# JeremyCCHsu/vae-npvc

Measured on AMD Instinct MI355X. Metric: SP frames/sec (train step: fwd+bwd+Adam), higher is better.
Workload: dtype f32 tensors and accumulation / bf16x2 operands (16 mantissa bits) on the matrix cores

## Files before the change

### include/vaenpvc.h

```cpp
#ifndef VAENPVC_H_
#define VAENPVC_H_

#include <stddef.h>
#include <stdint.h>

#ifdef __cplusplus
extern "C" {
#endif

#define VAENPVC_MAX_LAYERS 8

#define VAENPVC_OK 0
#define VAENPVC_E_ARG (-1)
#define VAENPVC_E_WORKSPACE (-2)
#define VAENPVC_E_HIP (-3)
#define VAENPVC_E_UNSUPPORTED (-4)
#define VAENPVC_E_STATE (-5)

#define VAENPVC_IMPL_AUTO 0
#define VAENPVC_IMPL_GENERIC 1

#define VAENPVC_MODE_INFER 0
#define VAENPVC_MODE_TRAIN 1

// ... 8 lines not shown
  int32_t y_dim;
  int32_t n_enc;
  int32_t enc_kernel[VAENPVC_MAX_LAYERS];
  int32_t enc_stride[VAENPVC_MAX_LAYERS];
  int32_t enc_output[VAENPVC_MAX_LAYERS];
  int32_t gen_h;
  int32_t gen_c;
  int32_t n_dec;
  int32_t dec_kernel[VAENPVC_MAX_LAYERS];
  int32_t dec_stride[VAENPVC_MAX_LAYERS];
  int32_t dec_output[VAENPVC_MAX_LAYERS];
} vaenpvc_arch;

typedef struct vaenpvc_ctx vaenpvc_ctx;

int vaenpvc_abi_version(void);
const char* vaenpvc_last_error(void);

int vaenpvc_ctx_create(const vaenpvc_arch* arch, vaenpvc_ctx** out);
void vaenpvc_ctx_destroy(vaenpvc_ctx* ctx);
int vaenpvc_set_impl(vaenpvc_ctx* ctx, int impl);
int vaenpvc_set_precision(vaenpvc_ctx* ctx, int planes);
int vaenpvc_get_precision(const vaenpvc_ctx* ctx);

int vaenpvc_param_count(const vaenpvc_ctx* ctx);
int64_t vaenpvc_param_floats(const vaenpvc_ctx* ctx);
int vaenpvc_param_info(const vaenpvc_ctx* ctx, int index, char* name, int name_cap,
                       int64_t* offset_floats, int32_t* ndim, int64_t* shape);

int64_t vaenpvc_workspace_bytes(const vaenpvc_ctx* ctx, int64_t F, int mode);
int vaenpvc_ws_find(const vaenpvc_ctx* ctx, int64_t F, int mode, const char* name,
                    int64_t* offset_floats, int64_t* count_floats);

int vaenpvc_encode_fwd(vaenpvc_ctx* ctx, const float* d_params, const float* d_x, int64_t F,
                       float* d_z_mu, float* d_z_lv, void* d_ws, size_t ws_bytes, void* stream);

int vaenpvc_decode_fwd(vaenpvc_ctx* ctx, const float* d_params, const float* d_z,
                       const int64_t* d_y, int64_t F, float* d_xh, void* d_ws, size_t ws_bytes,
                       void* stream);

int vaenpvc_train_fwd_bwd(vaenpvc_ctx* ctx, const float* d_params, const float* d_x,
                          const int64_t* d_y, const float* d_eps, int64_t F, float* d_grads,
                          float* d_loss3, void* d_ws, size_t ws_bytes, void* stream);

int vaenpvc_train_fwd_bwd_seeded(vaenpvc_ctx* ctx, const float* d_params, const float* d_x,
                                 const int64_t* d_y, uint64_t seed, uint64_t offset,
// ... 126 lines not shown
```

### vae-npvc_amd/csrc/abi.hip

```cpp
#include <climits>
#include <cmath>
#include <cstdarg>
#include <cstdio>
#include <cstring>
#include <map>
#include <memory>
#include <mutex>

#include "../../include/vaenpvc_debug.h"
#include "kernels.h"

using namespace vaenpvc;

typedef std::pair<std::vector<Region>, int64_t> Layout;
struct vaenpvc_ctx {
  Model m;
  int impl = VAENPVC_IMPL_AUTO;
  Runtime rt;
  std::recursive_mutex mu;
  std::map<std::pair<int64_t, int>, std::shared_ptr<const Layout>> ws_cache;
};
struct Call {
  std::lock_guard<std::recursive_mutex> lk;
  RtScope sc;
// ... 90 lines not shown

static bool use_tuned(const vaenpvc_ctx* c) {
  return c->impl == VAENPVC_IMPL_AUTO && c->m.is_vcc2016 && tuned::available();
}

extern "C" {

int vaenpvc_set_tuned_masks(vaenpvc_ctx* ctx, uint32_t fwd_mask, uint32_t bwd_mask) {
  if (!ctx) return fail(VAENPVC_E_ARG, "null context");
  Call call(ctx, false);
  ctx->rt.fwd_mask = fwd_mask;
  ctx->rt.bwd_mask = bwd_mask;
  return 0;
}

int vaenpvc_set_precision(vaenpvc_ctx* ctx, int planes) {
  if (!ctx || planes < 1 || planes > 3) return fail(VAENPVC_E_ARG, "precision must be 1, 2 or 3 bf16 terms");
  Call call(ctx, false);
  ctx->rt.planes = planes;
  return 0;
}
int vaenpvc_get_precision(const vaenpvc_ctx* ctx) { return ctx ? ctx->rt.planes : VAENPVC_E_ARG; }

int vaenpvc_set_bucket_callback(vaenpvc_ctx* ctx, vaenpvc_bucket_cb cb, void* user) {
  if (!ctx) return fail(VAENPVC_E_ARG, "null context");
  Call call(ctx, false);
  ctx->rt.bucket_cb = cb;
  ctx->rt.bucket_user = user;
  return 0;
}

int vaenpvc_timer_select(vaenpvc_ctx* ctx, const char* tag) {
  if (!ctx) return fail(VAENPVC_E_ARG, "null context");
  Call call(ctx, false);
  ctx->rt.tag = tag ? tag : "";
  ctx->rt.used = 0;
  return 0;
}

int vaenpvc_timer_read(vaenpvc_ctx* ctx, double* total_ms, int64_t* launches) {
  if (!ctx) return fail(VAENPVC_E_ARG, "null context");
  Call call(ctx, false);
  Runtime& r = ctx->rt;
  double tot = 0.0;
  for (size_t i = 0; i < r.used; ++i) {
    float ms = 0.f;
// ... 617 lines not shown
```

### vae-npvc_amd/csrc/gfx950_elem.h

```cpp
#pragma once
#include "gfx950_common.h"

namespace vaenpvc {
namespace tuned {

template <int N>
__global__ void __launch_bounds__(256) k_ln_stats_fast(const float* __restrict__ a, float* __restrict__ st, int F) {
  static_assert(N % 4 == 0, "frame size must be a multiple of 4 floats");
  constexpr int NV = N / 4, PER = cdiv(NV, 64);
  const int lane = threadIdx.x & 63;
  const int f = blockIdx.x * 4 + (threadIdx.x >> 6);
  if (f >= F) return;
  const float4* p = reinterpret_cast<const float4*>(a + (int64_t)f * N);
  float4 v[PER];
  float s = 0.f;
#pragma unroll
  for (int i = 0; i < PER; ++i) {
    int idx = lane + 64 * i;
    v[i] = idx < NV ? p[idx] : make_float4(0.f, 0.f, 0.f, 0.f);
    s += (v[i].x + v[i].y) + (v[i].z + v[i].w);
  }
  const float mean = wave_sum(s) / N;
  float q = 0.f;
#pragma unroll
// ... 729 lines not shown
    int yk[8];
#pragma unroll
    for (int u = 0; u < 8; ++u) {
      const int f = f0 + u < fe ? f0 + u : fe - 1;
      v[u] = f0 + u < fe ? d[(int64_t)f * N + nn] : 0.f;
      int64_t yy = y[f];
      yk[u] = (int)(yy < 0 ? 0 : (yy >= NY ? NY - 1 : yy));
    }
#pragma unroll
    for (int u = 0; u < 8; ++u) {
      const int ku = __builtin_amdgcn_readfirstlane(yk[u]);
#pragma unroll
      for (int k = 0; k < NY; ++k)
        if (ku == k) acc[k] += v[u];
    }
  }
  if (n < N) {
#pragma unroll
    for (int k = 0; k < NY; ++k)
      if (acc[k] != 0.f) atomicAdd(S + (int64_t)k * N + n, acc[k]);
  }
}

template <int NY>
__global__ void __launch_bounds__(256) k_merge_small(const float* __restrict__ S, const float* __restrict__ E,
                                                     const float* __restrict__ Wy, int zd, int M, float* __restrict__ dWy,
                                                     float* __restrict__ dE, float* __restrict__ db1, float* __restrict__ db2,
                                                     float* __restrict__ db3, int nb_w, int nb_e) {
  const int b = blockIdx.x, tid = threadIdx.x;
  if (b < nb_w) {
    const int i = b * 256 + tid;
    if (i >= zd * M) return;
    const int m = i / M, n = i - m * M;
    float acc = 0.f;
#pragma unroll
    for (int k = 0; k < NY; ++k) acc += E[k * zd + m] * S[(int64_t)k * M + n];
    dWy[i] = acc;
  } else if (b < nb_w + nb_e) {
    const int o = (b - nb_w) * 4 + (tid >> 6), lane = tid & 63;
    if (o >= NY * zd) return;
    const int k = o / zd, m = o - k * zd;
    float acc = 0.f;
    for (int n = lane; n < M; n += 64) acc += S[(int64_t)k * M + n] * Wy[(int64_t)m * M + n];
    acc = wave_sum(acc);
    if (lane == 0) dE[o] = acc;
  } else {
// ... 105 lines not shown
```

### vae-npvc_amd/csrc/gfx950_layers.hip

```cpp
#include <cstdlib>
#include <cstring>
#include <type_traits>

#include "gfx950_convgemm.h"
#include "gfx950_convwgrad.h"
#include "gfx950_dense.h"
#include "gfx950_elem.h"
#include "gfx950_tngemm.h"
#include "gfx950_toeplitz.h"
#include "gfx950_toep_bf16.h"
#include "gfx950_planegemm.h"
#include "gfx950_ntring.h"
#include "gfx950_viewconv.h"
#include "gfx950_fconv.h"
#include "gfx950_fwgrad.h"
#include "gfx950_fconv_r.h"
#include "gfx950_fbwd.h"
#include "gfx950_lnb_planes.h"
#include "kernels.h"

namespace vaenpvc {
namespace tuned {

#ifndef E1F_T
// ... 120 lines not shown
  static constexpr int gd2 = d2f + D2F::BTOTAL;
  static constexpr int gd0 = gd2 + GD2::BTOTAL;
  static constexpr int ge4 = gd0 + GD0::BTOTAL;
  static constexpr int ge3 = ge4 + GE4::BTOTAL;
  static constexpr int ge2 = ge3 + GE3::BTOTAL;
  static constexpr int ge1 = ge2 + GE2::BTOTAL;
  static constexpr int wc = ge1 + GE1::BTOTAL;
  static constexpr int lnpart = wc + TOEP_C * WROW;
  static constexpr int wdg = lnpart + 2048 * 3 * 256;
  static constexpr int wfw = wdg + TB_WFLOATS;
  static constexpr int heads_bias = wfw + TB_WFLOATS;
  static constexpr int pg_headsf = heads_bias + 256;
  static constexpr int pg_headsb = pg_headsf + 3 * 256 * 768 / 2;
  static constexpr int pg_mergef = pg_headsb + 3 * 768 * 256 / 2;
  static constexpr int pg_mergeb = pg_mergef + 3 * 1664 * 128 / 2;
  static constexpr int pg_enc4f = pg_mergeb + 3 * 128 * 1600 / 2;
  static constexpr int pg_enc4b = pg_enc4f + 3 * 768 * 896 / 2;
  static constexpr int pg_bias4 = pg_enc4b + 3 * 896 * 768 / 2;
  static constexpr int cvw = pg_bias4 + 768;
  static constexpr int cvwr_d0f = cvw + CV_WTOTAL;
  static constexpr int cvwr_e2g = cvwr_d0f + fcr_wfloats(CV_D0F);
  static constexpr int enc0part_ = cvwr_e2g + fcr_wfloats(CV_E2G);
  static constexpr int enc0part = enc0part_;
  static constexpr int total = enc0part + 512 * 7 * 16;
};
static_assert(Pk::total <= 8 * 939162 + 65536, "packed weights must fit the scratch region");
static inline bool sel(unsigned mask, int bit) { return (mask >> bit) & 1u; }
static inline bool fwd_on(int bit) { return sel(rt().fwd_mask, bit); }
static inline bool bwd_on(int bit) { return sel(rt().bwd_mask, bit); }
constexpr unsigned SEL_STEPS = (2u << VAENPVC_SEL_DEC3) - 1;
constexpr int64_t PLANEGEMM_MIN_FRAMES = 1024;
static inline bool pg_on(unsigned mask, int64_t F) {
  return sel(mask, VAENPVC_SEL_PLANE_GEMM) && (F >= PLANEGEMM_MIN_FRAMES || !sel(mask, VAENPVC_SEL_PLANE_GEMM_MIN_FRAMES));
}
static inline bool pg_fwd(int64_t F) { return pg_on(rt().fwd_mask, F); }
static inline bool cg_fwd(int64_t F) { return fwd_on(VAENPVC_SEL_VIEW_GEMM) && pg_on(rt().fwd_mask | (1u << VAENPVC_SEL_PLANE_GEMM), F); }
static inline bool cg_bwd(int64_t F) { return bwd_on(VAENPVC_SEL_VIEW_GEMM) && pg_on(rt().bwd_mask | (1u << VAENPVC_SEL_PLANE_GEMM), F); }
static inline bool pg_bwd(int64_t F) { return pg_on(rt().bwd_mask, F); }
static inline bool pg_step(int bit, int64_t F) { return bwd_on(bit) && pg_bwd(F) && pg_fwd(F) && fwd_on(bit); }
static inline bool cv_sel(unsigned mask, int site) { return !sel(mask, VAENPVC_SEL_CV_SITE_SET) || ((rt().cv_sites() >> site) & 1u); }
static inline bool cv_fwd(int site, int64_t F) { return cg_fwd(F) && cv_sel(rt().fwd_mask, site); }
static inline bool cv_bwd(int site, int64_t F) { return cg_bwd(F) && cv_sel(rt().bwd_mask, site); }
constexpr int64_t FCONV_MIN_FRAMES = 1024;
constexpr int64_t ENC0_WAVE_MIN_FRAMES = 1024;
static inline bool enc0_wave(unsigned mask, int64_t F) { return F >= ENC0_WAVE_MIN_FRAMES || !sel(mask, VAENPVC_SEL_ENC0_WAVE_MIN_FRAMES); }
static inline bool fc_on(unsigned mask, int site, int64_t F) {
  if (!fconv_serves(site, rt().planes)) return false;
// ... 18 lines not shown
  if (rt().planes > VAENPVC_FB_MAXPL || !bwd_on(VAENPVC_SEL_FBWD)) return false;
  if (!((rt().fb_layers() >> layer) & 1u)) return false;
  return F >= FCONV_MIN_FRAMES || !bwd_on(VAENPVC_SEL_FBWD_MIN_FRAMES);
}
static bool toep_bf16_for(int64_t F);
static inline bool act_bf16(int64_t F) {
  Runtime& r = rt();
  if (!r.act_bf16 || r.planes != 1 || F < FCONV_MIN_FRAMES) return false;
  const unsigned need = (1u << VAENPVC_SEL_DEC1) | (1u << VAENPVC_SEL_DEC2) | (1u << VAENPVC_SEL_DEC3);
  if ((r.fwd_mask & need) != need || (r.bwd_mask & need) != need) return false;
  return fc_fwd(CV_D1F, F) && fc_fwd(CV_D2F, F) && toep_bf16_for(F) && fb_bwd(FB_D2, F) && fb_bwd(FB_D1, F);
}
static inline bool fc_any(int64_t F) {
  for (int i = 0; i < CV_COUNT; ++i)
    if (fc_fwd(i, F) || fc_bwd(i, F) || fcr_fwd(i, F) || fcr_bwd(i, F)) return true;
  return false;
}
static inline bool fwd_planes(int bit, int site, int64_t F) {
  return fwd_on(bit) && cv_fwd(site, F) && !fc_fwd(site, F) && !fcr_fwd(site, F);
}
static inline bool cw_bwd(int site, int64_t F) { return cg_bwd(F) && cv_sel(rt().bwd_mask, CV_COUNT + site); }
static inline bool d0f_leaves_planes(int64_t F) {
  return F >= 1024 && fwd_on(VAENPVC_SEL_DEC0) && fcr_fwd(CV_D0F, F) && bwd_on(VAENPVC_SEL_DEC0) && cw_bwd(CW_D0, F);
}
static inline unsigned short* us(float* p) { return reinterpret_cast<unsigned short*>(p); }
static NtArgs nt_args(const float* Ap, int M, int Kp, const float* Bp, int Np, int N, float* C, int ldc) {
  NtArgs a;
  memset(&a, 0, sizeof a);
  a.A = reinterpret_cast<const unsigned short*>(Ap);
  a.B = reinterpret_cast<const unsigned short*>(Bp);
  a.a_plane = (int64_t)M * Kp;
  a.b_plane = (int64_t)Np * Kp;
  a.M = M;
  a.N = N;
  a.Kp = Kp;
  a.C = C;
  a.ldc = ldc;
  return a;
}
#ifndef TN_WGS_DENSE
#define TN_WGS_DENSE 384
#endif
static TnpArgs tnp_args(const float* Ap, int lda, const float* Bp, int ldb, int M, int N, int F, float* C, int ldc) {
  TnpArgs a;
  memset(&a, 0, sizeof a);
  a.A = reinterpret_cast<const unsigned short*>(Ap);
// ... 305 lines not shown
    a.beta = P + m.enc[4].beta_off;
    a.out2 = w.z_lv;
    a.split = 128;
    a.bias = w.scratch + Pk::heads_bias;
    if (F < SMALL_BATCH_FRAMES) {
      if (w.z_lv == w.z_mu + (size_t)F * 128) {
        (void)hipMemsetAsync(w.z_mu, 0, (size_t)F * 256 * 4, s);
      } else {
        (void)hipMemsetAsync(w.z_mu, 0, (size_t)F * 128 * 4, s);
        (void)hipMemsetAsync(w.z_lv, 0, (size_t)F * 128 * 4, s);
      }
      VAENPVC_TIMED("heads_fwd", s, launch_densegemm<HeadsFs>(a, s, 6));
    } else
    VAENPVC_TIMED("heads_fwd", s, launch_densegemm<HeadsF>(a, s));
  } else generic::heads_fwd(m, P, F, w, s);
}

void decoder_fwd(const Model& m, const float* P, const float* z, const int64_t* y, int64_t F64, const Ws& w,
                 float* xh_out, hipStream_t s, bool weights_packed) {
  const int F = (int)F64;
  if (!weights_packed) prep(m, P, w, F, s);
  const bool z_planes_done = rt().plz_F == F && z == w.z;
  rt().plz_F = -1;
  if (fwd_on(VAENPVC_SEL_MERGE) && pg_fwd(F)) {
    for_planes([&](auto npl) {
      constexpr int NPL = decltype(npl)::value;
      if (!z_planes_done) VAENPVC_TIMED("merge_split", s, launch_split<NPL>(split_args(z, 128, 128, F, us(w.pl_z)), s));
      NtArgs a = nt_args(w.pl_z, F, 128, w.scratch + Pk::pg_mergef, 1664, 1539, w.h, 1539);
      a.rowbias = w.scratch + Pk::merge_tb;
      a.idx = y;
      a.nrb = MERGE_NY;
      a.ldrb = 1539;
      VAENPVC_TIMED("merge_fwd", s, launch_gemm_nt<NPL>(a, s));
    });
  } else if (fwd_on(VAENPVC_SEL_MERGE)) {
    DenseArgs a = dense_args(z, w.scratch + Pk::merge_f, w.h, m.merge, F);
    a.idx = y;
    a.rowbias = w.scratch + Pk::merge_tb;
    a.nrb = MERGE_NY;
    VAENPVC_TIMED("merge_fwd", s, (F < SMALL_BATCH_FRAMES ? launch_densegemm<MergeFs>(a, s) : launch_densegemm<MergeF>(a, s)));
  } else generic::merge_fwd(m, P, z, y, F, w, s);
  const bool abf = act_bf16(F);
  auto fused = [&](int site, const float* src, const float* st, float* st_out, const ConvL* ln, const float* bias, float* out, const char* tag,
                   bool bf_in = false, bool bf_out = false) {
    for_planes([&](auto npl) {
      FcArgs fa{src, st, st_out, ln ? P + ln->gamma_off : nullptr, ln ? P + ln->beta_off : nullptr,
// ... 7 lines not shown
    for_planes([&](auto npl) {
      constexpr int NPL = decltype(npl)::value;
      if (have) {}
      else if (i == 0) VAENPVC_TIMED(tsplit, s, cv_split<NPL>(cl, src, nullptr, nullptr, nullptr, w.cl[cl], F, s));
      else VAENPVC_TIMED(tsplit, s, cv_split<NPL>(cl, src, w.dec_st[i - 1], P + m.dec[i - 1].gamma_off, P + m.dec[i - 1].beta_off, w.cl[cl], F, s));
      VAENPVC_TIMED(tgemm, s, cv_gemm<NPL>(site, w.scratch + Pk::cvw + cv_woff(site), w.cl[cl], w.dec_a[i], P + m.dec[i].b_off, F, s));
    });
  };
  auto dec_stats = [&](int i, int next_site, int cl, const char* tag) {
    const bool fuse = fwd_on(VAENPVC_SEL_DEC1 + i) && cv_fwd(next_site, F) && !fc_fwd(next_site, F);
    if (fuse)
      for_planes([&](auto npl) {
        VAENPVC_TIMED(tag, s, cv_stats_split<decltype(npl)::value>(cl, w.dec_a[i], w.dec_st[i], P + m.dec[i].gamma_off, P + m.dec[i].beta_off,
                                                                   w.cl[cl], F, s));
      });
    return fuse;
  };
  bool have_yd0 = false, have_yd1 = false;
  const bool d1_fused = fwd_on(VAENPVC_SEL_DEC1) && fc_fwd(CV_D1F, F), d2_fused = fwd_on(VAENPVC_SEL_DEC2) && fc_fwd(CV_D2F, F);
  if (fwd_on(VAENPVC_SEL_DEC0) && fcr_fwd(CV_D0F, F)) {
    for_planes([&](auto npl) {
      FcArgs fa{w.h, nullptr, nullptr, nullptr, nullptr, reinterpret_cast<const unsigned short*>(w.scratch + Pk::cvwr_d0f),
                P + m.dec[0].b_off, w.dec_a[0], F};
      if (w.d_h && d0f_leaves_planes(F)) {
        fa.cl_out = us(w.cl[CL_H]);
        fa.cl_plane = cl_plane(CL_H, F);
      }
      VAENPVC_TIMED("dec0_fwd", s, fconv_r<decltype(npl)::value>(CV_D0F, fa, s));
    });
    if (!d1_fused && !(have_yd0 = dec_stats(0, CV_D1F, CL_YD0, "dec1_split"))) VAENPVC_TIMED("stats_dec0", s, stats<1824>(w.dec_a[0], w.dec_st[0], F, s));
  } else if (fwd_on(VAENPVC_SEL_DEC0) && cv_fwd(CV_D0F, F)) {
    dec_view(CV_D0F, CL_H, 0, false, w.h, "dec0_split", "dec0_fwd");
    if (!d1_fused && !(have_yd0 = dec_stats(0, CV_D1F, CL_YD0, "dec1_split"))) VAENPVC_TIMED("stats_dec0", s, stats<1824>(w.dec_a[0], w.dec_st[0], F, s));
  } else if (fwd_on(VAENPVC_SEL_DEC0)) {
    VAENPVC_TIMED("dec0_fwd", s, (F < SMALL_BATCH_FRAMES ? launch_convgemm<D0Fs>(conv_args(w.h, nullptr, nullptr, nullptr, w.scratch + Pk::d0f,
                                                                P + m.dec[0].b_off, w.dec_a[0], F), nsplit_for<D0Fs>(F), s) : launch_convgemm<D0F>(conv_args(w.h, nullptr, nullptr, nullptr, w.scratch + Pk::d0f,
                                                                P + m.dec[0].b_off, w.dec_a[0], F), nsplit_for<D0F>(F), s)));
    if (!d1_fused && !(have_yd0 = dec_stats(0, CV_D1F, CL_YD0, "dec1_split"))) VAENPVC_TIMED("stats_dec0", s, stats<1824>(w.dec_a[0], w.dec_st[0], F, s));
  } else generic::dec_layer_fwd(m, P, F, w, xh_out, s, 0);
  if (fwd_on(VAENPVC_SEL_DEC1) && fc_fwd(CV_D1F, F)) {
    fused(CV_D1F, w.dec_a[0], nullptr, w.dec_st[0], &m.dec[0], P + m.dec[1].b_off, w.dec_a[1], "dec1_fwd", false, abf);
    if (!d2_fused && !(have_yd1 = dec_stats(1, CV_D2F, CL_YD1, "dec2_split"))) VAENPVC_TIMED("stats_dec1", s, stats<2736>(w.dec_a[1], w.dec_st[1], F, s));
  } else if (fwd_on(VAENPVC_SEL_DEC1) && cv_fwd(CV_D1F, F)) {
    dec_view(CV_D1F, CL_YD0, 1, have_yd0, w.dec_a[0], "dec1_split", "dec1_fwd");
    if (!d2_fused && !(have_yd1 = dec_stats(1, CV_D2F, CL_YD1, "dec2_split"))) VAENPVC_TIMED("stats_dec1", s, stats<2736>(w.dec_a[1], w.dec_st[1], F, s));
  } else if (fwd_on(VAENPVC_SEL_DEC1)) {
    VAENPVC_TIMED("dec1_fwd", s, launch_convgemm<D1F>(conv_args(w.dec_a[0], w.dec_st[0], P + m.dec[0].gamma_off,
                                                                P + m.dec[0].beta_off, w.scratch + Pk::d1f,
                                                                P + m.dec[1].b_off, w.dec_a[1], F), nsplit_for<D1F>(F), s));
// ... 136 lines not shown
  return (toep_bf16_for(F) && bwd_on(VAENPVC_SEL_DEC2) && bwd_on(VAENPVC_SEL_DEC3) && fb_bwd(FB_D2, F) && !act_bf16(F) && !frame_bwd_on(F)) ? DY2_PITCH : TB_H;
}
bool loss_fwd_post(const Model& m, const float* P, const float* x, int64_t F64, const Ws& w, float* loss3, hipStream_t s) {
  const int F = (int)F64;
  if (!w.d_xh || !w.toep_gp || !w.dy_tmp || !w.dec_y || !w.d_dec_a[0] || !fwd_on(VAENPVC_SEL_DEC2) || !fwd_on(VAENPVC_SEL_DEC3) || F < 1024 || frame_bwd_on(F64) || !bwd_on(VAENPVC_SEL_DEC3) || !toep_bf16_for(F) || act_bf16(F)) return false;
  for_planes([&](auto npl) {
    constexpr int NPL = decltype(npl)::value;
    hipLaunchKernelGGL((k_nll_dxh_post<NPL>), dim3((unsigned)nll_post_blocks(F)), dim3(256), 0, s, x, w.xh, w.nll_f,
                       rt().dxh_skip && toep_wgrad_bf16_for(F) ? nullptr : w.d_xh, P + m.dec[3].w_off,
                       reinterpret_cast<unsigned short*>(w.toep_gp), w.dy_tmp, w.scratch + Pk::lnpart, F, 1.0f / (float)F, w.dec_y,
                       w.d_dec_a[0],
                       dy2_pitch(F));
  });
  generic::loss_reduce(F, w, loss3, s);
  rt().dxh_post_F = F;
  return true;
}

void backward(const Model& m, const float* P, const float* x, const int64_t* y, const float* eps, int64_t F64,
              const Ws& w, float* G, hipStream_t s) {
  const int F = (int)F64;
  const bool abf = act_bf16(F64);
  (void)hipMemsetAsync(G, 0, (size_t)m.n_params * 4, s);
  hipStream_t side = bwd_on(VAENPVC_SEL_WGRAD_STREAM) && (F < SIDE_STREAM_MAX_FRAMES || rt().planes != 2 || rt().side_forced) ? rt().side_stream() : nullptr;
  const bool fork = side != nullptr;
  hipStream_t s2 = fork ? side : s;
  auto ready = [&]() { if (fork) rt().stream_dep(s, s2); };
  auto bucket = [&](int64_t off, int64_t end) {
    Runtime& r = rt();
    if (!r.bucket_cb) return;
    ready();
    r.bucket_cb(r.bucket_user, r.bucket_next++, off, end - off, (void*)s2);
  };
  const bool toep_planes = bwd_on(VAENPVC_SEL_DEC3) && toep_bf16_for(F);
  const bool post_done = toep_planes && rt().dxh_post_F == F;
  rt().dxh_post_F = -1;
  if (post_done)
    VAENPVC_TIMED("dxh_post", s, hipLaunchKernelGGL(k_colsum_part, dim3(1), dim3(256), 0, s, w.scratch + Pk::lnpart, nll_post_blocks(F), 1, G + m.dec[3].b_off);
                  hipLaunchKernelGGL(k_sum_parts_add, dim3((unsigned)cdiv(513 * 8, 64)), dim3(1024), 0, s, w.d_dec_a[0], nll_post_blocks(F), 513 * 8, G + m.dec[3].w_off));
  else if (toep_planes)
    for_planes([&](auto npl) {
      constexpr int NPL_ = decltype(npl)::value;
      auto launch_dp = [&](auto kern) {
        VAENPVC_TIMED("dxh_post", s, hipLaunchKernelGGL(kern, dim3((unsigned)cmin_(2048, cdiv((int)F, 4))), dim3(256), 0, s, w.d_xh, P + m.dec[3].w_off,
                           reinterpret_cast<unsigned short*>(w.toep_gp), w.dy_tmp, G + m.dec[3].b_off, (int)F, dy2_pitch(F)));
      };
// ... 233 lines not shown
    dec_bias_done[0] = true;
  } else if (bwd_on(VAENPVC_SEL_DEC1)) {
    const ConvL &l = m.dec[1], &pl = m.dec[0];
    WgArgs a{w.d_dec_a[1], nullptr, nullptr, nullptr, w.dec_a[0], w.dec_st[0], P + pl.gamma_off, P + pl.beta_off,
             G + l.w_off, F, 0};
    const bool fg = fc_bwd(CV_D1G, F), vg = !fg && cv_bwd(CV_D1G, F), fw = fw_bwd(CW_D1, F), vw = !fw && cw_bwd(CW_D1, F);
    if (vg || vw) gsplit(CL_GD1, w.d_dec_a[1], "dec1_gsplit");
    if (vw && !fwd_planes(VAENPVC_SEL_DEC1, CV_D1F, F)) asplit(CL_YD0, w.dec_a[0], w.dec_st[0], &pl, "dec1_asplit");
    ready();
    if (fw) fwg(CW_D1, w.dec_a[0], w.dec_st[0], &pl, w.d_dec_a[1], nullptr, nullptr, G + l.w_off, "dec1_wgrad");
    else if (vw) vwgrad(CW_D1, G + l.w_off, "dec1_wgrad");
    else VAENPVC_TIMED("dec1_wgrad", s2, launch_convwgrad<WD1>(a, WGS, s2));
    if (!dec_bias_done[1]) generic::bias_grad(w.d_dec_a[1], G + l.b_off, F, l.cout, l.hout, s);
    if (fg) fdgrad(CV_D1G, w.d_dec_a[1], w.dy_tmp, "dec1_dgrad");
    else if (vg) vdgrad(CV_D1G, w.dy_tmp, "dec1_dgrad");
    else
    VAENPVC_TIMED("dec1_dgrad", s, launch_convgemm<GD1>(conv_args(w.d_dec_a[1], nullptr, nullptr, nullptr, P + l.w_off, nullptr,
                                                                  w.dy_tmp, F), nsplit_for<GD1>(F), s));
    lnb_dec0(w.dy_tmp);
    dec_bias_done[0] = true;
  } else generic::bwd_dec_layer(m, P, F, w, G, s, 1);

  const bool dh_planes = rt().d0g_planes && gd0_only_planes && fcr_otl(CV_D0G, rt().planes) && pg_step(VAENPVC_SEL_MERGE, F) && F >= 64;
  if (bwd_on(VAENPVC_SEL_DEC0)) {
    const ConvL& l = m.dec[0];
    WgArgs a{w.d_dec_a[0], nullptr, nullptr, nullptr, w.h, nullptr, nullptr, nullptr, G + l.w_off, F, 0};
    const bool rg = fcr_bwd(CV_D0G, F), vg = !rg && cv_bwd(CV_D0G, F), vw = cw_bwd(CW_D0, F);
    if ((vg || vw) && !gd0_planes) gsplit(CL_GD0, w.d_dec_a[0], "dec0_gsplit");
    if (vw && !fwd_planes(VAENPVC_SEL_DEC0, CV_D0F, F) && !d0f_leaves_planes(F)) asplit(CL_H, w.h, nullptr, nullptr, "dec0_asplit");
    ready();
    if (vw) vwgrad(CW_D0, G + l.w_off, "dec0_wgrad");
    else VAENPVC_TIMED("dec0_wgrad", s2, launch_convwgrad<WD0>(a, WGS, s2));
    if (!dec_bias_done[0]) generic::bias_grad(w.d_dec_a[0], G + l.b_off, F, l.cout, l.hout, s);
    if (rg) rdgrad(CV_D0G, w.scratch + Pk::cvw + cv_woff(CV_D0G), w.d_dec_a[0], w.d_h, "dec0_dgrad", gd0_only_planes ? w.cl[CL_GD0] : nullptr,
                   dh_planes ? w.pl_dh : nullptr, 1600);
    else if (vg) vdgrad(CV_D0G, w.d_h, "dec0_dgrad");
    else
    VAENPVC_TIMED("dec0_dgrad", s, (F < SMALL_BATCH_FRAMES ? launch_convgemm<GD0s>(conv_args(w.d_dec_a[0], nullptr, nullptr, nullptr, w.scratch + Pk::gd0,
                                                                  nullptr, w.d_h, F), nsplit_for<GD0s>(F), s) : launch_convgemm<GD0>(conv_args(w.d_dec_a[0], nullptr, nullptr, nullptr, w.scratch + Pk::gd0,
                                                                  nullptr, w.d_h, F), nsplit_for<GD0>(F), s)));
  } else generic::bwd_dec_layer(m, P, F, w, G, s, 0);
  if (lnq) flush_ln_reduce(*lnq, s);
  bucket(m.dec[0].w_off, m.n_params);

  if (bwd_on(VAENPVC_SEL_MERGE)) {
    const bool pgm = pg_step(VAENPVC_SEL_MERGE, F);
    if (pgm) {
      for_planes([&](auto npl) {
        constexpr int NPL = decltype(npl)::value;
        if (F >= 64) {
        int nch = 0;
        if (dh_planes) VAENPVC_TIMED("merge_dsplit", s, (nch = launch_segsum_planes<NPL, MERGE_NY>(us(w.pl_dh), (int64_t)F * 1600, y, 1539, 1600, F, w.dy_tmp, s)));
        else
        VAENPVC_TIMED("merge_dsplit", s, (nch = launch_split_segsum<NPL, MERGE_NY>(w.d_h, y, 1539, 1600, F, us(w.pl_dh), w.dy_tmp, s)));
        VAENPVC_TIMED("merge_segsum", s, launch_sum_parts(w.dy_tmp, nch, MERGE_NY * 1539, w.scratch + Pk::merge_s, s));
        } else {
        SplitArgs sa = split_args(w.d_h, 1539, 1600, F, us(w.pl_dh));
        VAENPVC_TIMED("merge_dsplit", s, launch_split<NPL>(sa, s));
        }
        ready();
        TnpArgs t = tnp_args(w.pl_z, 128, w.pl_dh, 1600, 128, 1539, F, G + m.wz_off, 1539);
        t.tn4 = bwd_on(VAENPVC_SEL_TN_W4);
        VAENPVC_TIMED("merge_wgrad", s2, (launch_gemm_tn<NPL, TN_EPI_PLAIN>(t, TN_WGS_DENSE, s2)));
      });
    } else {
    TnArgs a = tn_args(w.z, 128, w.d_h, 1539, 128, 1539, F, G + m.wz_off, 1539);
    ready();
    VAENPVC_TIMED("merge_wgrad", s2, launch_tngemm(a, false, kchunks_for(F, 13), s2));
    }
    float* Sg = w.scratch + Pk::merge_s;
    if (!(pgm && F >= 64)) {
      (void)hipMemsetAsync(Sg, 0, (size_t)MERGE_NY * 1539 * 4, s);
      int ch = cmax(1, cmin_(cdiv(F, 64), 128)), fc = cdiv(F, ch);
      VAENPVC_TIMED("merge_segsum", s, hipLaunchKernelGGL(k_segsum_atomic<MERGE_NY>, dim3((unsigned)cdiv(1539, 256), (unsigned)cdiv(F, fc)), dim3(256), 0, s,
                                                          w.d_h, y, 1539, F, fc, Sg));
    }
    const int nb_w = cdiv(128 * 1539, 256), nb_e = cdiv(MERGE_NY * 128, 4), nb_b = cdiv(1539, 256);
    VAENPVC_TIMED("merge_small", s, hipLaunchKernelGGL(k_merge_small<MERGE_NY>, dim3((unsigned)(nb_w + nb_e + nb_b)), dim3(256), 0, s, Sg, P + m.emb_off, P + m.wy_off, 128,
                       1539, G + m.wy_off, G + m.emb_off, G + m.bz_off, G + m.by_off, G + m.bm_off, nb_w, nb_e));
    if (pgm) {
      for_planes([&](auto npl) {
        constexpr int NPL = decltype(npl)::value;
        NtArgs a = nt_args(w.pl_dh, F, 1600, w.scratch + Pk::pg_mergeb, 128, 128, w.d_z, 128);
        VAENPVC_TIMED("merge_dgrad", s, launch_gemm_nt<NPL>(a, s));
      });
    } else {
      DenseArgs d = dense_args(w.d_h, w.scratch + Pk::merge_b, w.d_z, 128, F);
      if (F < SMALL_BATCH_FRAMES) {
        (void)hipMemsetAsync(w.d_z, 0, (size_t)F * 128 * 4, s);
        VAENPVC_TIMED("merge_dgrad", s, launch_densegemm<MergeBs>(d, s, 7));
      } else
      VAENPVC_TIMED("merge_dgrad", s, launch_densegemm<MergeB>(d, s));
    }
  } else generic::bwd_merge(m, P, y, F, w, G, s);
// ... 332 lines not shown
```

### vae-npvc_amd/csrc/runtime.h

```cpp
#pragma once
#include <hip/hip_runtime.h>

#include <cstdint>
#include <cstring>
#include <string>
#include <unordered_set>
#include <utility>
#include <vector>

namespace vaenpvc {

struct Runtime {
  unsigned fwd_mask = 0xffffffffu, bwd_mask = 0xffffffffu;
  int planes = 2;
  unsigned cv_sites() const { return planes == 1 ? 0xe2ceu : planes == 2 ? 0xc244u : 0x4u; }
  static constexpr unsigned FC_SITES = 0xdb1u;
  static constexpr unsigned FCR_SITES = 0x28au;
  static constexpr unsigned FW_SITES = 0x3fu;
  long fb_layers_env = -1;
  unsigned fb_layers() const { return fb_layers_env >= 0 ? (unsigned)fb_layers_env : 0x7u; }
  bool act_bf16 = false;
  int nt_ar = 0;
  int nt_ring = 1;
  int cg_sf_ring = 1;
  int cg_pf_ring = 0;
  bool dxh_skip = true;
  bool d0g_planes = true;
  int d2_lna = 1;
  bool d2_tail = false;
  bool toep_f32 = false;
  bool side_enabled = true;
  bool side_forced = false;
  int frame_max = 512;
  int64_t last_F = -1;
  int last_path = -1, last_planes = 0;
  unsigned last_fwd_mask = 0, last_bwd_mask = 0;
  const void* last_ws = nullptr;
  int64_t plz_F = -1;
  int64_t dxh_post_F = -1;
  int device = -1;
  hipStream_t s2 = nullptr;
  hipEvent_t ev[16] = {};
  int ev_next = 0;
  std::unordered_set<const void*> attr_done;
  void (*bucket_cb)(void* user, int32_t bucket, int64_t off, int64_t cnt, void* ready_stream) = nullptr;
  void* bucket_user = nullptr;
  int bucket_next = 0;
  std::string tag;
  std::vector<std::pair<hipEvent_t, hipEvent_t>> pool;
  size_t used = 0;

  void read_env();
  void bind_device();
  void release();
  void ensure_lds(const void* fn, int bytes);
  hipStream_t side_stream();
  void stream_dep(hipStream_t from, hipStream_t to);

  bool timer_match(const char* t) const {
    if (tag.empty()) return false;
    const size_t n = strlen(t);
    for (size_t p = tag.find(t); p != std::string::npos; p = tag.find(t, p + 1))
// ... 16 lines not shown
```

### vae-npvc_amd/csrc/runtime.hip

```cpp
#include "runtime.h"

#include <cstdlib>
#include <cstring>

namespace vaenpvc {

static thread_local Runtime* tl_rt = nullptr;
static Runtime g_detached;

Runtime& rt() { return tl_rt ? *tl_rt : g_detached; }
RtScope::RtScope(Runtime* r) : prev(tl_rt) { tl_rt = r; }
RtScope::~RtScope() { tl_rt = prev; }

void Runtime::read_env() {
  if (const char* e = getenv("VAENPVC_FWD_MASK")) fwd_mask = (unsigned)strtoul(e, nullptr, 0);
  if (const char* e = getenv("VAENPVC_BWD_MASK")) bwd_mask = (unsigned)strtoul(e, nullptr, 0);
  if (const char* e = getenv("VAENPVC_SIDE_STREAM")) {
    side_enabled = e[0] != '0';
    side_forced = side_enabled;
  }
  if (const char* e = getenv("VAENPVC_TOEP")) toep_f32 = !strcmp(e, "f32");
  if (const char* e = getenv("VAENPVC_D2_TAIL")) d2_tail = atoi(e) != 0;
  if (const char* e = getenv("VAENPVC_D2_LNA")) d2_lna = atoi(e);
  if (const char* e = getenv("VAENPVC_D0G_PLANES")) d0g_planes = atoi(e) != 0;
  if (const char* e = getenv("VAENPVC_DXH_SKIP")) dxh_skip = atoi(e) != 0;
  if (const char* e = getenv("VAENPVC_NT_RING")) nt_ring = atoi(e);
  if (const char* e = getenv("VAENPVC_CG_SF_RING")) cg_sf_ring = atoi(e);
  if (const char* e = getenv("VAENPVC_CG_PF_RING")) cg_pf_ring = atoi(e);
  if (const char* e = getenv("VAENPVC_NT_AR")) nt_ar = atoi(e);
  if (const char* e = getenv("VAENPVC_FRAME_MAX")) frame_max = atoi(e) < 0 ? 0 : (atoi(e) > 1024 ? 1024 : atoi(e));
  if (const char* e = getenv("VAENPVC_FB_LAYERS")) fb_layers_env = (long)strtoul(e, nullptr, 0);
  if (const char* e = getenv("VAENPVC_ACT_BF16")) act_bf16 = atoi(e) != 0;
  if (const char* e = getenv("VAENPVC_PLANES")) {
    int p = atoi(e);
    if (p >= 1 && p <= 3) planes = p;
  }
}

void Runtime::release() {
  if (s2) {
    (void)hipStreamSynchronize(s2);
    (void)hipStreamDestroy(s2);
    for (auto& e : ev)
      if (e) (void)hipEventDestroy(e);
  }
  s2 = nullptr;
  for (auto& e : ev) e = nullptr;
  ev_next = 0;
  for (auto& p : pool) {
    (void)hipEventDestroy(p.first);
    (void)hipEventDestroy(p.second);
  }
// ... 62 lines not shown
```

### vae-npvc_amd/hipvae/engine.py

```python
import ctypes as C
import math
from collections import OrderedDict

import torch

from . import lib as L


def arch_to_struct(arch):
    a = L.Arch()
    enc, gen = arch['encoder'], arch['generator']
    for net in (enc, gen):
        assert len(net['output']) == len(net['kernel']) == len(net['stride'])
    if len(enc['output']) > L.MAX_LAYERS or len(gen['output']) > L.MAX_LAYERS:
        raise ValueError('at most %d layers per net' % L.MAX_LAYERS)
    a.H = int(arch['hwc'][0])
    if int(arch['hwc'][1]) != 1 or int(arch['hwc'][2]) != 1:
        raise ValueError('frame-wise model: hwc must be [H, 1, 1]')
    a.z_dim, a.y_dim = int(arch['z_dim']), int(arch['y_dim'])
    a.n_enc = len(enc['output'])
    for i, (o, k, s) in enumerate(zip(enc['output'], enc['kernel'], enc['stride'])):
        if int(k[1]) != 1 or int(s[1]) != 1:
            raise ValueError('kernels/strides must be [k, 1]')
        a.enc_output[i], a.enc_kernel[i], a.enc_stride[i] = int(o), int(k[0]), int(s[0])
# ... 59 lines not shown
        self._loss3 = torch.zeros(3, dtype=torch.float32, device=self.device)
        self._flag = torch.zeros(1, dtype=torch.int32, device=self.device)
        self._bucket_cb = None

    def __del__(self):
        try:
            if getattr(self, 'ctx', None):
                self.lib.vaenpvc_ctx_destroy(self.ctx)
                self.ctx = None
        except Exception:
            pass

    def set_impl(self, impl):
        code = {'auto': L.IMPL_AUTO, 'generic': L.IMPL_GENERIC}.get(impl, impl)
        L.check(self.lib.vaenpvc_set_impl(self.ctx, int(code)), 'set_impl')

    def set_precision(self, precision):
        code = L.PRECISIONS.get(precision, precision)
        L.check(self.lib.vaenpvc_set_precision(self.ctx, int(code)), 'set_precision')

    @property
    def precision(self):
        return int(self.lib.vaenpvc_get_precision(self.ctx))

    def set_tuned_masks(self, fwd=0xffffffff, bwd=0xffffffff):
        L.check(self.lib.vaenpvc_set_tuned_masks(self.ctx, fwd & 0xffffffff, bwd & 0xffffffff), 'set_tuned_masks')

    def timer_select(self, tag):
        L.check(self.lib.vaenpvc_timer_select(self.ctx, tag.encode() if tag else None), 'timer_select')

    def timer_read(self):
        ms, n = C.c_double(), C.c_int64()
        L.check(self.lib.vaenpvc_timer_read(self.ctx, C.byref(ms), C.byref(n)), 'timer_read')
        return ms.value, n.value

    def set_bucket_callback(self, fn):
        if fn is None:
            L.check(self.lib.vaenpvc_set_bucket_callback(self.ctx, L.BUCKET_CB(), None), 'set_bucket_callback')
            self._bucket_cb = None
            return
        thunk = L.BUCKET_CB(lambda user, b, off, cnt, stream: fn(int(b), int(off), int(cnt), stream))
        L.check(self.lib.vaenpvc_set_bucket_callback(self.ctx, thunk, None), 'set_bucket_callback')
        self._bucket_cb = thunk

    def _query_layout(self):
        out = OrderedDict()
# ... 299 lines not shown
```

### vae-npvc_amd/hipvae/lib.py

```python
import ctypes as C
import os
import subprocess

_HERE = os.path.dirname(os.path.abspath(__file__))
CSRC = os.path.normpath(os.path.join(_HERE, '..', 'csrc'))
LIB_PATH = os.environ.get('VAENPVC_LIB') or os.path.join(CSRC, 'libvaenpvc_hip.so')
MAX_LAYERS = 8
ABI_VERSION = 4

MODE_INFER, MODE_TRAIN = 0, 1
IMPL_AUTO, IMPL_GENERIC = 0, 1
PREC_BF16X3, PREC_BF16X2, PREC_BF16 = 3, 2, 1
PRECISIONS = {'auto': 2, 'bf16x2': 2, 'bf16x3': 3, 'bf16': 1}
SEL_ENC0 = 0
SEL_ENC1 = 1
SEL_ENC2 = 2
SEL_ENC3 = 3
SEL_ENC4 = 4
SEL_HEADS = 5
SEL_MERGE = 6
SEL_DEC0 = 7
SEL_DEC1 = 8
SEL_DEC2 = 9
SEL_DEC3 = 10
# ... 70 lines not shown
    'vaenpvc_gv_postfilter': (C.c_int, [_P, _P, _I32, _I64, _I32, _P, _P, _P, _P, _P, C.c_size_t, _P]),
    'vaenpvc_synth_workspace_bytes': (_I64, [_I32, _I64, _I32, _I32]),
    'vaenpvc_synthesize': (C.c_int, [_P, _P, _P, _P, _P, _P, _I32, _I64, _I64, _I32, _I32, C.c_double, _U64, _P, _P,
                                     C.c_size_t, _P]),
    'vaenpvc_analysis_workspace_bytes': (_I64, [_I32, _I64, _I64, _I32, C.c_double, C.c_double, C.c_double]),
    'vaenpvc_analyze': (C.c_int, [_P, _P, _P, _I32, _I64, _I64, _I32, C.c_double, C.c_double, C.c_double, _P, _P, _P, _P,
                                  _P, C.c_size_t, _P]),
    'vaenpvc_mcep_matrix': (C.c_int, [_I32, C.c_double, _I32, _P]),
    'vaenpvc_mcd_workspace_bytes': (_I64, [_I32, _I64, _I64, _I64, _I32]),
    'vaenpvc_mcd_dtw': (C.c_int, [_P, _P, _P, _P, _I64, _P, _P, _P, _P, _I64, _I32, _I64, _P, _I32, _P, _P, _P, _P,
                                  C.c_size_t, _P]),
    'vaenpvc_column_select_workspace_bytes': (_I64, [_I64, _I32, _I32]),
    'vaenpvc_column_select': (C.c_int, [_P, _I64, _I32, _I64, _P, _I32, _P, _P, _P, C.c_size_t, _P]),
    'vaenpvc_speaker_stats_workspace_bytes': (_I64, [_I64, _I32, _I32]),
    'vaenpvc_speaker_stats': (C.c_int, [_P, _I64, _P, _I64, _P, _P, _I32, _I32, _I64, _I32, _P, _P, _P, _P, C.c_size_t,
                                        _P]),
    'vaenpvc_resample_plan': (C.c_int, [_I32, _I32, C.POINTER(_I32), C.POINTER(_I32), C.POINTER(_I32)]),
    'vaenpvc_resample_filter': (C.c_int, [_I32, _I32, _P]),
    'vaenpvc_resample': (C.c_int, [_P, _P, _P, _I32, _I64, _I64, _I32, _I32, _P, _P, _P]),
    'vaenpvc_unpack_records': (C.c_int, [_P, _I64, _I32, _I32, _P, _P, _P, _P, _P]),
    'vaenpvc_gather_unpack_records': (C.c_int, [_P, _I64, _P, _I64, _I32, _I32, _P, _P, _P, _P, _P]),
    'vaenpvc_set_precision': (C.c_int, [_P, C.c_int]),
    'vaenpvc_get_precision': (C.c_int, [_P]),
    'vaenpvc_train_fwd_bwd_seeded': (C.c_int, [_P, _P, _P, _P, _U64, _U64, _P, _I64, _P, _P, _P, C.c_size_t, _P]),
    'vaenpvc_loss_fwd_seeded': (C.c_int, [_P, _P, _P, _P, _U64, _U64, _I64, _P, _P, C.c_size_t, _P]),
    'vaenpvc_philox_normal': (C.c_int, [_U64, _U64, _P, _I64, _P]),
    'vaenpvc_set_bucket_callback': (C.c_int, [_P, BUCKET_CB, _P]),
    'vaenpvc_validate_ids': (C.c_int, [_P, _P, _I64, _P, _P]),
    'vaenpvc_summary': (C.c_int, [_P, _I64, _P, _I32, _P, _P, _P]),
    'vaenpvc_philox_uniform': (C.c_int, [_U64, _U64, _P, _I64, _P]),
    'vaenpvc_train_fwd_bwd_target': (C.c_int, [_P, _P, _P, _P, _P, _P, _I64, _P, _P, _P, C.c_size_t, _P]),
    'vaenpvc_train_bwd_target': (C.c_int, [_P, _P, _P, _P, _P, _P, _I64, _P, _P, _P, C.c_size_t, _P]),
    'vaenpvc_disc_create': (C.c_int, [C.POINTER(DiscArch), C.POINTER(_P)]),
    'vaenpvc_disc_destroy': (None, [_P]),
    'vaenpvc_disc_param_count': (C.c_int, [_P]),
    'vaenpvc_disc_param_floats': (_I64, [_P]),
    'vaenpvc_disc_param_info': (C.c_int, [_P, C.c_int, C.c_char_p, C.c_int, C.POINTER(_I64), C.POINTER(_I32),
                                          C.POINTER(_I64)]),
    'vaenpvc_disc_workspace_bytes': (_I64, [_P, _I64]),
    'vaenpvc_disc_fwd': (C.c_int, [_P, _P, _P, _P, _I64, _P, _P, _P, C.c_size_t, _P]),
    'vaenpvc_disc_critic_fwd_bwd': (C.c_int, [_P, _P, _P, _P, _P, _I64, _F, _P, _P, _P, C.c_size_t, _P]),
    'vaenpvc_disc_generator_target': (C.c_int, [_P, _P, _P, _P, _I64, _F, _P, _P, _P, C.c_size_t, _P]),
}

_lib = None

# ... 37 lines not shown
```

Before: 5.831 million.

## Factorise decoder-0 weight gradient through latent and speaker embedding products

Result: faster. 5.915 million (median of 6 runs) (+1.4%).

```diff
diff --git a/include/vaenpvc.h b/include/vaenpvc.h
--- a/include/vaenpvc.h
+++ b/include/vaenpvc.h
@@ -54,6 +54,12 @@
 int vaenpvc_set_impl(vaenpvc_ctx* ctx, int impl);
 int vaenpvc_set_precision(vaenpvc_ctx* ctx, int planes);
 int vaenpvc_get_precision(const vaenpvc_ctx* ctx);
+#define VAENPVC_D0W_ROUTE_FP32 0
+#define VAENPVC_D0W_ROUTE_FACTOR 1
+#define VAENPVC_D0W_ROUTE_PLANES 2
+#define VAENPVC_D0W_ROUTE_PLANES_REDO 3
+int vaenpvc_set_d0w_factor(vaenpvc_ctx* ctx, int mode);
+int vaenpvc_get_d0w_route(const vaenpvc_ctx* ctx);
 
 int vaenpvc_param_count(const vaenpvc_ctx* ctx);
 int64_t vaenpvc_param_floats(const vaenpvc_ctx* ctx);
diff --git a/vae-npvc_amd/csrc/abi.hip b/vae-npvc_amd/csrc/abi.hip
--- a/vae-npvc_amd/csrc/abi.hip
+++ b/vae-npvc_amd/csrc/abi.hip
@@ -136,6 +136,14 @@
 }
 int vaenpvc_get_precision(const vaenpvc_ctx* ctx) { return ctx ? ctx->rt.planes : VAENPVC_E_ARG; }
 
+int vaenpvc_set_d0w_factor(vaenpvc_ctx* ctx, int mode) {
+  if (!ctx || mode < 0 || mode > 2) return fail(VAENPVC_E_ARG, "d0w factor mode must be 0, 1 or 2");
+  Call call(ctx, false);
+  ctx->rt.d0w_factor = mode;
+  return 0;
+}
+int vaenpvc_get_d0w_route(const vaenpvc_ctx* ctx) { return ctx ? ctx->rt.d0w_route : VAENPVC_E_ARG; }
+
 int vaenpvc_set_bucket_callback(vaenpvc_ctx* ctx, vaenpvc_bucket_cb cb, void* user) {
   if (!ctx) return fail(VAENPVC_E_ARG, "null context");
   Call call(ctx, false);
diff --git a/vae-npvc_amd/csrc/gfx950_elem.h b/vae-npvc_amd/csrc/gfx950_elem.h
--- a/vae-npvc_amd/csrc/gfx950_elem.h
+++ b/vae-npvc_amd/csrc/gfx950_elem.h
@@ -775,6 +775,15 @@
   }
 }
 
+__global__ void __launch_bounds__(256) k_cl_rows_to_frames(const float* __restrict__ src, float* __restrict__ dst, int rows, int C, int H,
+                                                           int CP, int HLO, int HP) {
+  const int n = rows * H * C;
+  for (int i = blockIdx.x * 256 + threadIdx.x; i < n; i += gridDim.x * 256) {
+    const int c = i % C, t = i / C, p = t % H, r = t / H;
+    dst[((int64_t)r * C + c) * H + p] = src[((int64_t)r * HP + HLO + p) * CP + c];
+  }
+}
+
 template <int NY>
 __global__ void __launch_bounds__(256) k_merge_small(const float* __restrict__ S, const float* __restrict__ E,
                                                      const float* __restrict__ Wy, int zd, int M, float* __restrict__ dWy,
diff --git a/vae-npvc_amd/csrc/gfx950_layers.hip b/vae-npvc_amd/csrc/gfx950_layers.hip
--- a/vae-npvc_amd/csrc/gfx950_layers.hip
+++ b/vae-npvc_amd/csrc/gfx950_layers.hip
@@ -166,7 +166,10 @@
   static constexpr int cvwr_e2g = cvwr_d0f + fcr_wfloats(CV_D0F);
   static constexpr int enc0part_ = cvwr_e2g + fcr_wfloats(CV_E2G);
   static constexpr int enc0part = enc0part_;
-  static constexpr int total = enc0part + 512 * 7 * 16;
+  static constexpr int d0w_c = enc0part + 512 * 7 * 16;
+  static constexpr int d0w_s = d0w_c + 128 * 2016;
+  static constexpr int d0w_y = d0w_s + MERGE_NY * 2016;
+  static constexpr int total = d0w_y + (128 + MERGE_NY) * 1824;
 };
 static_assert(Pk::total <= 8 * 939162 + 65536, "packed weights must fit the scratch region");
 static inline bool sel(unsigned mask, int bit) { return (mask >> bit) & 1u; }
@@ -231,6 +234,12 @@
 static inline bool cw_bwd(int site, int64_t F) { return cg_bwd(F) && cv_sel(rt().bwd_mask, CV_COUNT + site); }
 static inline bool d0f_leaves_planes(int64_t F) {
   return F >= 1024 && fwd_on(VAENPVC_SEL_DEC0) && fcr_fwd(CV_D0F, F) && bwd_on(VAENPVC_SEL_DEC0) && cw_bwd(CW_D0, F);
+}
+constexpr int64_t D0W_FACTOR_MIN_FRAMES = 1024;
+static inline bool d0w_factor_on(int64_t F) {
+  const int mode = rt().d0w_factor;
+  if (mode <= 0 || (mode == 1 && F < D0W_FACTOR_MIN_FRAMES)) return false;
+  return bwd_on(VAENPVC_SEL_DEC0) && cw_bwd(CW_D0, F) && bwd_on(VAENPVC_SEL_MERGE) && pg_step(VAENPVC_SEL_MERGE, F);
 }
 static inline unsigned short* us(float* p) { return reinterpret_cast<unsigned short*>(p); }
 static NtArgs nt_args(const float* Ap, int M, int Kp, const float* Bp, int Np, int N, float* C, int ldc) {
@@ -582,6 +591,7 @@
   if (!weights_packed) prep(m, P, w, F, s);
   const bool z_planes_done = rt().plz_F == F && z == w.z;
   rt().plz_F = -1;
+  rt().clh_F = -1;
   if (fwd_on(VAENPVC_SEL_MERGE) && pg_fwd(F)) {
     for_planes([&](auto npl) {
       constexpr int NPL = decltype(npl)::value;
@@ -635,9 +645,10 @@
     for_planes([&](auto npl) {
       FcArgs fa{w.h, nullptr, nullptr, nullptr, nullptr, reinterpret_cast<const unsigned short*>(w.scratch + Pk::cvwr_d0f),
                 P + m.dec[0].b_off, w.dec_a[0], F};
-      if (w.d_h && d0f_leaves_planes(F)) {
+      if (w.d_h && d0f_leaves_planes(F) && !d0w_factor_on(F)) {
         fa.cl_out = us(w.cl[CL_H]);
         fa.cl_plane = cl_plane(CL_H, F);
+        rt().clh_F = F;
       }
       VAENPVC_TIMED("dec0_fwd", s, fconv_r<decltype(npl)::value>(CV_D0F, fa, s));
     });
@@ -820,6 +831,7 @@
   const int F = (int)F64;
   const bool abf = act_bf16(F64);
   (void)hipMemsetAsync(G, 0, (size_t)m.n_params * 4, s);
+  rt().d0w_route = VAENPVC_D0W_ROUTE_FP32;
   hipStream_t side = bwd_on(VAENPVC_SEL_WGRAD_STREAM) && (F < SIDE_STREAM_MAX_FRAMES || rt().planes != 2 || rt().side_forced) ? rt().side_stream() : nullptr;
   const bool fork = side != nullptr;
   hipStream_t s2 = fork ? side : s;
@@ -1099,14 +1111,60 @@
   } else generic::bwd_dec_layer(m, P, F, w, G, s, 1);
 
   const bool dh_planes = rt().d0g_planes && gd0_only_planes && fcr_otl(CV_D0G, rt().planes) && pg_step(VAENPVC_SEL_MERGE, F) && F >= 64;
+  const bool d0w = d0w_factor_on(F);
+  static_assert(CLD[CL_GD0].HP * CLD[CL_GD0].CP == 2016 && CLD[CL_GD0].C * CLD[CL_GD0].H == 1824 && GD0s::KC * GD0s::HIN == 1824 && GD0s::N * GD0s::HOUT == 1539,
+                "pseudo-frames of the factorised route");
+  constexpr int D0W_ROW = 2016, D0W_FR = 1824;
+  float* const d0w_ys = w.scratch + Pk::d0w_y + 128 * D0W_FR;
+  auto d0w_unpack = [&](const float* src, float* dst, int rows, const char* tag, hipStream_t st) {
+    const ClDesc& d = CLD[CL_GD0];
+    VAENPVC_TIMED(tag, st, hipLaunchKernelGGL(k_cl_rows_to_frames, dim3((unsigned)cdiv(rows * D0W_FR, 256)), dim3(256), 0, st, src, dst, rows,
+                                                       d.C, d.H, d.CP, d.HLO, d.HP));
+  };
+  auto d0w_sums = [&]() {
+    float* Sc = w.scratch + Pk::d0w_s;
+    for_planes([&](auto npl) {
+      constexpr int NPL = decltype(npl)::value;
+      const bool one = F < 64;
+      int nch = 0;
+      VAENPVC_TIMED("merge_segsum", s, (nch = launch_segsum_planes<NPL, MERGE_NY>(us(w.cl[CL_GD0]), cl_plane(CL_GD0, F), y, D0W_ROW, D0W_ROW, F,
+                                                                                  one ? Sc : w.dy_tmp, s)));
+      if (!one) VAENPVC_TIMED("merge_segsum", s, launch_sum_parts(w.dy_tmp, nch, MERGE_NY * D0W_ROW, Sc, s));
+    });
+    d0w_unpack(Sc, d0w_ys, MERGE_NY, "merge_segsum", s);
+    VAENPVC_TIMED("merge_wgrad", s, launch_convgemm<GD0s>(conv_args(d0w_ys, nullptr, nullptr, nullptr, w.scratch + Pk::gd0, nullptr,
+                                                                    w.scratch + Pk::merge_s, MERGE_NY), nsplit_for<GD0s>(MERGE_NY), s));
+  };
+  auto d0w_wgrads = [&]() {
+    float* Wc = w.scratch + Pk::d0w_c;
+    float* Yc = w.scratch + Pk::d0w_y;
+    (void)hipMemsetAsync(Wc, 0, (size_t)128 * D0W_ROW * 4, s2);
+    for_planes([&](auto npl) {
+      constexpr int NPL = decltype(npl)::value;
+      TnpArgs t = tnp_args(w.pl_z, 128, w.cl[CL_GD0], D0W_ROW, 128, D0W_ROW, F, Wc, D0W_ROW);
+      t.b_plane = cl_plane(CL_GD0, F);
+      VAENPVC_TIMED("dec0_wgrad", s2, (launch_gemm_tn<NPL, TN_EPI_PLAIN>(t, TN_WGS_DENSE, s2)));
+    });
+    d0w_unpack(Wc, Yc, 128, "dec0_wgrad", s2);
+    const ConvL& l = m.dec[0];
+    WgArgs az{Yc, nullptr, nullptr, nullptr, P + m.wz_off, nullptr, nullptr, nullptr, G + l.w_off, 128, 0};
+    WgArgs ay{d0w_ys, nullptr, nullptr, nullptr, w.scratch + Pk::merge_tb, nullptr, nullptr, nullptr, G + l.w_off, MERGE_NY, 0};
+    VAENPVC_TIMED("dec0_wgrad", s2, launch_convwgrad<WD0>(az, WGS, s2); launch_convwgrad<WD0>(ay, WGS, s2));
+    VAENPVC_TIMED("merge_wgrad", s2, launch_convgemm<GD0s>(conv_args(Yc, nullptr, nullptr, nullptr, w.scratch + Pk::gd0, nullptr, G + m.wz_off, 128),
+                                                           nsplit_for<GD0s>(128), s2));
+  };
   if (bwd_on(VAENPVC_SEL_DEC0)) {
     const ConvL& l = m.dec[0];
     WgArgs a{w.d_dec_a[0], nullptr, nullptr, nullptr, w.h, nullptr, nullptr, nullptr, G + l.w_off, F, 0};
     const bool rg = fcr_bwd(CV_D0G, F), vg = !rg && cv_bwd(CV_D0G, F), vw = cw_bwd(CW_D0, F);
     if ((vg || vw) && !gd0_planes) gsplit(CL_GD0, w.d_dec_a[0], "dec0_gsplit");
-    if (vw && !fwd_planes(VAENPVC_SEL_DEC0, CV_D0F, F) && !d0f_leaves_planes(F)) asplit(CL_H, w.h, nullptr, nullptr, "dec0_asplit");
+    const bool h_planes = fwd_planes(VAENPVC_SEL_DEC0, CV_D0F, F) || (d0f_leaves_planes(F) && rt().clh_F == F);
+    if (vw && !d0w && !h_planes) asplit(CL_H, w.h, nullptr, nullptr, "dec0_asplit");
+    rt().d0w_route = d0w ? VAENPVC_D0W_ROUTE_FACTOR : !vw ? VAENPVC_D0W_ROUTE_FP32 : h_planes ? VAENPVC_D0W_ROUTE_PLANES : VAENPVC_D0W_ROUTE_PLANES_REDO;
+    if (d0w) d0w_sums();
     ready();
-    if (vw) vwgrad(CW_D0, G + l.w_off, "dec0_wgrad");
+    if (d0w) d0w_wgrads();
+    else if (vw) vwgrad(CW_D0, G + l.w_off, "dec0_wgrad");
     else VAENPVC_TIMED("dec0_wgrad", s2, launch_convwgrad<WD0>(a, WGS, s2));
     if (!dec_bias_done[0]) generic::bias_grad(w.d_dec_a[0], G + l.b_off, F, l.cout, l.hout, s);
     if (rg) rdgrad(CV_D0G, w.scratch + Pk::cvw + cv_woff(CV_D0G), w.d_dec_a[0], w.d_h, "dec0_dgrad", gd0_only_planes ? w.cl[CL_GD0] : nullptr,
@@ -1125,6 +1183,10 @@
     if (pgm) {
       for_planes([&](auto npl) {
         constexpr int NPL = decltype(npl)::value;
+        if (d0w) {
+          if (!dh_planes) VAENPVC_TIMED("merge_dsplit", s, launch_split<NPL>(split_args(w.d_h, 1539, 1600, F, us(w.pl_dh)), s));
+          return;
+        }
         if (F >= 64) {
         int nch = 0;
         if (dh_planes) VAENPVC_TIMED("merge_dsplit", s, (nch = launch_segsum_planes<NPL, MERGE_NY>(us(w.pl_dh), (int64_t)F * 1600, y, 1539, 1600, F, w.dy_tmp, s)));
@@ -1146,7 +1208,7 @@
     VAENPVC_TIMED("merge_wgrad", s2, launch_tngemm(a, false, kchunks_for(F, 13), s2));
     }
     float* Sg = w.scratch + Pk::merge_s;
-    if (!(pgm && F >= 64)) {
+    if (!(pgm && F >= 64) && !d0w) {
       (void)hipMemsetAsync(Sg, 0, (size_t)MERGE_NY * 1539 * 4, s);
       int ch = cmax(1, cmin_(cdiv(F, 64), 128)), fc = cdiv(F, ch);
       VAENPVC_TIMED("merge_segsum", s, hipLaunchKernelGGL(k_segsum_atomic<MERGE_NY>, dim3((unsigned)cdiv(1539, 256), (unsigned)cdiv(F, fc)), dim3(256), 0, s,
diff --git a/vae-npvc_amd/csrc/runtime.h b/vae-npvc_amd/csrc/runtime.h
--- a/vae-npvc_amd/csrc/runtime.h
+++ b/vae-npvc_amd/csrc/runtime.h
@@ -31,6 +31,7 @@
   bool toep_f32 = false;
   bool side_enabled = true;
   bool side_forced = false;
+  int d0w_factor = 1;
   int frame_max = 512;
   int64_t last_F = -1;
   int last_path = -1, last_planes = 0;
@@ -38,6 +39,8 @@
   const void* last_ws = nullptr;
   int64_t plz_F = -1;
   int64_t dxh_post_F = -1;
+  int64_t clh_F = -1;
+  int d0w_route = 0;
   int device = -1;
   hipStream_t s2 = nullptr;
   hipEvent_t ev[16] = {};
diff --git a/vae-npvc_amd/csrc/runtime.hip b/vae-npvc_amd/csrc/runtime.hip
--- a/vae-npvc_amd/csrc/runtime.hip
+++ b/vae-npvc_amd/csrc/runtime.hip
@@ -28,6 +28,7 @@
   if (const char* e = getenv("VAENPVC_CG_SF_RING")) cg_sf_ring = atoi(e);
   if (const char* e = getenv("VAENPVC_CG_PF_RING")) cg_pf_ring = atoi(e);
   if (const char* e = getenv("VAENPVC_NT_AR")) nt_ar = atoi(e);
+  if (const char* e = getenv("VAENPVC_D0W_FACTOR")) d0w_factor = atoi(e) < 0 ? 0 : (atoi(e) > 2 ? 2 : atoi(e));
   if (const char* e = getenv("VAENPVC_FRAME_MAX")) frame_max = atoi(e) < 0 ? 0 : (atoi(e) > 1024 ? 1024 : atoi(e));
   if (const char* e = getenv("VAENPVC_FB_LAYERS")) fb_layers_env = (long)strtoul(e, nullptr, 0);
   if (const char* e = getenv("VAENPVC_ACT_BF16")) act_bf16 = atoi(e) != 0;
diff --git a/vae-npvc_amd/hipvae/engine.py b/vae-npvc_amd/hipvae/engine.py
--- a/vae-npvc_amd/hipvae/engine.py
+++ b/vae-npvc_amd/hipvae/engine.py
@@ -105,6 +105,13 @@
     @property
     def precision(self):
         return int(self.lib.vaenpvc_get_precision(self.ctx))
+
+    def set_d0w_factor(self, mode):
+        L.check(self.lib.vaenpvc_set_d0w_factor(self.ctx, int(mode)), 'set_d0w_factor')
+
+    @property
+    def d0w_route(self):
+        return int(self.lib.vaenpvc_get_d0w_route(self.ctx))
 
     def set_tuned_masks(self, fwd=0xffffffff, bwd=0xffffffff):
         L.check(self.lib.vaenpvc_set_tuned_masks(self.ctx, fwd & 0xffffffff, bwd & 0xffffffff), 'set_tuned_masks')
diff --git a/vae-npvc_amd/hipvae/lib.py b/vae-npvc_amd/hipvae/lib.py
--- a/vae-npvc_amd/hipvae/lib.py
+++ b/vae-npvc_amd/hipvae/lib.py
@@ -116,6 +116,8 @@
     'vaenpvc_gather_unpack_records': (C.c_int, [_P, _I64, _P, _I64, _I32, _I32, _P, _P, _P, _P, _P]),
     'vaenpvc_set_precision': (C.c_int, [_P, C.c_int]),
     'vaenpvc_get_precision': (C.c_int, [_P]),
+    'vaenpvc_set_d0w_factor': (C.c_int, [_P, C.c_int]),
+    'vaenpvc_get_d0w_route': (C.c_int, [_P]),
     'vaenpvc_train_fwd_bwd_seeded': (C.c_int, [_P, _P, _P, _P, _U64, _U64, _P, _I64, _P, _P, _P, C.c_size_t, _P]),
     'vaenpvc_loss_fwd_seeded': (C.c_int, [_P, _P, _P, _P, _U64, _U64, _I64, _P, _P, C.c_size_t, _P]),
     'vaenpvc_philox_normal': (C.c_int, [_U64, _U64, _P, _I64, _P]),
```
